# visanalexandru/felics

Hardware: AMD Instinct MI355X
Metric: encode MPix/s on 4K 8-bit grayscale batch (bit-exact); % HBM-read roofline (higher is better)
Workload: dtype u8

## Files before the change

### felics_amd/csrc/felics_kernels.hip

```cpp
#include <hip/hip_runtime.h>
#include <stdint.h>
#include <stdlib.h>
#include <string.h>
#include <type_traits>

#include "felics_device.h"
#include "felics_kernels.h"
#include "felics_codes.h"
#include "felics_pairs.h"

namespace felics {

thread_local LaunchTiming g_launch_timing;


__device__ __forceinline__ void ycocg(int r, int gr, int b, int &yv, int &co, int &cg) {
    co = r - b;
    const int t = b + co / 2;
    cg = gr - t;
    yv = t + cg / 2;
}

__device__ __forceinline__ void rgb8_group(const uint8_t *__restrict__ src, int16_t *__restrict__ o, uint32_t i, uint32_t npix, uint64_t stride) {
    if (i + 4 <= npix) {
        uint32_t w[3];
        __builtin_memcpy(w, src, 12);
        int yv[4], co[4], cg[4];
        ycocg((int)(w[0] & 0xFFu), (int)((w[0] >> 8) & 0xFFu), (int)((w[0] >> 16) & 0xFFu), yv[0], co[0], cg[0]);
        ycocg((int)(w[0] >> 24), (int)(w[1] & 0xFFu), (int)((w[1] >> 8) & 0xFFu), yv[1], co[1], cg[1]);
        ycocg((int)((w[1] >> 16) & 0xFFu), (int)(w[1] >> 24), (int)(w[2] & 0xFFu), yv[2], co[2], cg[2]);
        ycocg((int)((w[2] >> 8) & 0xFFu), (int)((w[2] >> 16) & 0xFFu), (int)(w[2] >> 24), yv[3], co[3], cg[3]);
        auto put4 = [&](int16_t *dst, const int (&v)[4]) {
            const uint32_t p[2] = {(uint32_t)(v[0] & 0xFFFF) | ((uint32_t)v[1] << 16),
                                   (uint32_t)(v[2] & 0xFFFF) | ((uint32_t)v[3] << 16)};
            __builtin_memcpy(dst, p, 8);
        };
        put4(o + i, yv);
        put4(o + stride + i, co);
        put4(o + 2ull * stride + i, cg);
    } else {
        for (uint32_t j = i; j < npix; j++) {
            int yv, co, cg;
            ycocg(src[(j - i) * 3], src[(j - i) * 3 + 1], src[(j - i) * 3 + 2], yv, co, cg);
            o[j] = (int16_t)yv;
            o[stride + j] = (int16_t)co;
            o[2ull * stride + j] = (int16_t)cg;
        }
    }
}
__global__ __launch_bounds__(256) void k_rgb8_to_planes(const uint8_t *__restrict__ rgb, int16_t *__restrict__ planes,
                                                        uint32_t npix, uint32_t nimg) {
    const uint32_t groups = (npix + 3) / 4;
    const uint64_t total = (uint64_t)groups * nimg;
    for (uint64_t g = (uint64_t)blockIdx.x * blockDim.x + threadIdx.x; g < total;
         g += (uint64_t)gridDim.x * blockDim.x) {
        const uint32_t img = (uint32_t)(g / groups);
        const uint32_t i = (uint32_t)(g - (uint64_t)img * groups) * 4;
        rgb8_group(rgb + ((uint64_t)img * npix + i) * 3, planes + (uint64_t)img * 3 * npix, i, npix, (uint64_t)npix);
    }
}
__global__ __launch_bounds__(256) void k_rgb8_to_planes_mixed(const PlaneGeom *__restrict__ table, uint64_t plane_stride) {
    const PlaneGeom *pg = table + 3ull * blockIdx.y;
    const uint32_t npix = pg->npix, groups = (npix + 3) / 4;
    const uint8_t *rgb = (const uint8_t *)pg->image;
    int16_t *o = (int16_t *)pg->samples;
    for (uint32_t g = blockIdx.x * blockDim.x + threadIdx.x; g < groups; g += gridDim.x * blockDim.x)
        rgb8_group(rgb + (uint64_t)g * 12u, o, g * 4, npix, plane_stride);
}

__global__ __launch_bounds__(256) void k_rgb8_view_to_planes(const PlaneGeom *__restrict__ table, const ViewRow *__restrict__ rows, uint64_t plane_stride) {
    const PlaneGeom *pg = table + 3ull * blockIdx.y;
    const ViewRow vr = rows[blockIdx.y];
    const uint32_t npix = pg->npix, W = pg->W, groups = (npix + 3) / 4;
    const uint8_t *data = (const uint8_t *)vr.data;
    const int64_t rs = vr.row_stride, ps = vr.pixel_stride, cs = vr.channel_stride;
    int16_t *o = (int16_t *)pg->samples;
    const bool unit = cs == 1 || cs == -1;
    const uint32_t mode = unit && ps == 3 ? 1u : unit && ps == 4 ? 2u : ps == 1 ? 3u : 0u;
    const uint8_t *low = data + (cs < 0 ? 2 * cs : 0);
    for (uint32_t g = blockIdx.x * blockDim.x + threadIdx.x; g < groups; g += gridDim.x * blockDim.x) {
        const uint32_t i = g * 4;
        uint32_t y = i / W, x = i - y * W;
        int r[4] = {0, 0, 0, 0}, gr[4] = {0, 0, 0, 0}, b[4] = {0, 0, 0, 0};
        const bool whole = i + 4 <= npix;
        const bool in_row = whole && x + 4 <= W && !(mode == 2u && x + 4 == W);
        if (in_row && mode == 1u) {
            uint32_t w[3];
            __builtin_memcpy(w, low + (int64_t)y * rs + (int64_t)x * 3, 12);
            const int q[12] = {(int)(w[0] & 0xFFu), (int)((w[0] >> 8) & 0xFFu), (int)((w[0] >> 16) & 0xFFu), (int)(w[0] >> 24),
                               (int)(w[1] & 0xFFu), (int)((w[1] >> 8) & 0xFFu), (int)((w[1] >> 16) & 0xFFu), (int)(w[1] >> 24),
                               (int)(w[2] & 0xFFu), (int)((w[2] >> 8) & 0xFFu), (int)((w[2] >> 16) & 0xFFu), (int)(w[2] >> 24)};
#pragma unroll
            for (uint32_t k = 0; k < 4; k++) {
                r[k] = cs > 0 ? q[3 * k] : q[3 * k + 2];
                gr[k] = q[3 * k + 1];
                b[k] = cs > 0 ? q[3 * k + 2] : q[3 * k];
            }
        } else if (in_row && mode == 2u) {
            uint32_t w[4];
            __builtin_memcpy(w, low + (int64_t)y * rs + (int64_t)x * 4, 16);
#pragma unroll
            for (uint32_t k = 0; k < 4; k++) {
                const int c0 = (int)(w[k] & 0xFFu), c2 = (int)((w[k] >> 16) & 0xFFu);
                r[k] = cs > 0 ? c0 : c2;
                gr[k] = (int)((w[k] >> 8) & 0xFFu);
                b[k] = cs > 0 ? c2 : c0;
            }
        } else if (in_row && mode == 3u) {
            const uint8_t *p = data + (int64_t)y * rs + (int64_t)x;
            load4(p, r);
            load4(p + cs, gr);
            load4(p + 2 * cs, b);
        } else {
            for (uint32_t k = 0; k < 4 && i + k < npix; k++) {
                const uint8_t *p = data + (int64_t)y * rs + (int64_t)x * ps;
                r[k] = p[0];
                gr[k] = p[cs];
                b[k] = p[2 * cs];
                if (++x == W) {
                    x = 0;
                    y++;
                }
            }
        }
        int yv[4], co[4], cg[4];
#pragma unroll
        for (uint32_t k = 0; k < 4; k++) ycocg(r[k], gr[k], b[k], yv[k], co[k], cg[k]);
        if (whole) {
            auto put4 = [&](int16_t *dst, const int (&v)[4]) {
                const uint32_t pk[2] = {(uint32_t)(v[0] & 0xFFFF) | ((uint32_t)v[1] << 16), (uint32_t)(v[2] & 0xFFFF) | ((uint32_t)v[3] << 16)};
                __builtin_memcpy(dst, pk, 8);
            };
            put4(o + i, yv);
            put4(o + plane_stride + i, co);
            put4(o + 2ull * plane_stride + i, cg);
        } else {
            for (uint32_t k = 0; i + k < npix; k++) {
                o[i + k] = (int16_t)yv[k];
                o[plane_stride + i + k] = (int16_t)co[k];
                o[2ull * plane_stride + i + k] = (int16_t)cg[k];
            }
        }
    }
}

template <uint32_t TABLE>
__device__ __forceinline__ uint32_t bitop3(uint32_t a, uint32_t b, uint32_t c) {
    return __builtin_amdgcn_bitop3_b32(a, b, c, TABLE);
}
constexpr uint32_t BT_SEL = 0xE4;
constexpr uint32_t BT_OR_ANDN = 0xF4;
constexpr uint32_t BT_ANDN = 0x30;
constexpr uint32_t BT_OR3 = 0xFE;
constexpr uint32_t BT_SEL_NOT = 0x72;
constexpr uint32_t BT_NOR = 0x03;
constexpr uint32_t BT_OR_AND = 0xF8;
__device__ __forceinline__ uint32_t min_u16(uint32_t a, uint32_t b) {
    uint32_t r;
    asm("v_min_u16 %0, %1, %2" : "=v"(r) : "v"(a), "v"(b));
    return r;
}
__device__ __forceinline__ uint32_t max_u16(uint32_t a, uint32_t b) {
    uint32_t r;
    asm("v_max_u16 %0, %1, %2" : "=v"(r) : "v"(a), "v"(b));
    return r;
}
template <uint32_t N>
__device__ __forceinline__ uint32_t shl_u16(uint32_t a) {
    uint32_t r;
    asm("v_lshlrev_b16 %0, %1, %2" : "=v"(r) : "n"(N), "v"(a));
    return r;
}
__device__ __forceinline__ uint32_t twice(uint32_t a) {
    uint32_t r;
    asm("v_add_u32 %0, %1, %1" : "=v"(r) : "v"(a));
    return r;
}
__device__ __forceinline__ uint32_t vgpr_const(uint32_t v) {
    uint32_t r;
    asm("v_mov_b32 %0, %1" : "=v"(r) : "s"(v));
    return r;
}

__device__ __forceinline__ uint32_t field_at(const uint32_t *w, uint32_t j, uint8_t) {
    const uint32_t x = w[j >> 2];
    switch (j & 3u) {
        case 0: return x & 0xFFu;
        case 1: {
            uint32_t r;
            asm("v_lshrrev_b16 %0, 8, %1" : "=v"(r) : "v"(x));
            return r;
        }
        case 2: return (x >> 16) & 0xFFu;
        default: return x >> 24;
    }
}
__device__ __forceinline__ uint32_t field_at(const uint32_t *w, uint32_t j, int16_t) {
    const uint32_t x = w[j >> 1] ^ 0x80008000u;
    return (j & 1u) ? x >> 16 : x & 0xFFFFu;
}
__device__ __forceinline__ uint32_t field_of(int v, uint8_t) { return (uint32_t)v & 0xFFu; }
__device__ __forceinline__ uint32_t field_of(int v, int16_t) { return ((uint32_t)v ^ 0x8000u) & 0xFFFFu; }

#ifndef FELICS_FORMS
#define FELICS_FORMS 255
#endif
#ifndef FELICS_FRONT_WAVES
#define FELICS_FRONT_WAVES 6
#endif
template <typename T>
struct PlaneView {
    const T *pl;
    uint32_t W, H, npix;
};
template <typename T>
__device__ __forceinline__ PlaneView<T> plane_view(const T *planes, uint32_t plane, uint32_t W, uint32_t npix) {
    return PlaneView<T>{planes + (uint64_t)plane * npix, W, 0u, npix};
}
template <typename T>
__device__ __forceinline__ PlaneView<T> plane_view(const PlaneGeom *table, uint32_t plane, uint32_t, uint32_t) {
    return plane_view<T>((const T *)nullptr, plane, table);
}
template <typename T>
__device__ __forceinline__ PlaneView<T> plane_view(const T *, uint32_t plane, const PlaneGeom *table) {
    const PlaneGeom *pg = table + (uint32_t)__builtin_amdgcn_readfirstlane((int)plane);
    return PlaneView<T>{(const T *)pg->samples, pg->W, pg->H, pg->npix};
}

template <typename T>
__device__ __forceinline__ PlaneView<T> plane_view(const PitchedGeom *rows, uint32_t plane, uint32_t, uint32_t) {
    const PitchedGeom *pg = rows + (uint32_t)__builtin_amdgcn_readfirstlane((int)plane);
    return PlaneView<T>{(const T *)pg->g.samples, pg->g.W, pg->g.H, pg->g.npix};
}
template <typename S>
__device__ __forceinline__ uint64_t plane_pitch(S, uint32_t) { return 0; }
__device__ __forceinline__ uint64_t plane_pitch(const PitchedGeom *rows, uint32_t plane) {
    return rows[(uint32_t)__builtin_amdgcn_readfirstlane((int)plane)].pitch;
}
#ifdef FELICS_FRONT_STAMPS
__device__ unsigned long long g_front_stamps[256][16];
#define FSTAMP(i)                                                              \
    do {                                                                       \
        const unsigned long long now_ = __builtin_amdgcn_s_memtime();          \
        f_acc[i] += now_ - f_last;                                             \
        f_last = now_;                                                         \
    } while (0)
#define FSTAMP_ARRIVED(d, t)                                                                                                              \
    do {                                                                                                                                  \
        FSTAMP(4 + (d));                                                                                                                  \
        asm volatile("" ::"v"(t.cur[0]), "v"(t.cur[1]), "v"(t.cur[2]), "v"(t.cur[3]), "v"(t.up[0]), "v"(t.up[1]), "v"(t.up[2]), "v"(t.up[3]), \
                     "v"(t.left0));                                                                                                       \
        FSTAMP(d);                                                                                                                        \
    } while (0)
#else
#define FSTAMP(i)
#define FSTAMP_ARRIVED(d, t)
#endif
template <typename T, typename ET, typename S, bool BALLOT>
__attribute__((amdgpu_waves_per_eu(sizeof(T) == 1 ? FELICS_FRONT_WAVES : 5))) __global__ __launch_bounds__(256) void k_front(
    S __restrict__ planes, ET *__restrict__ ev, uint16_t *__restrict__ pix, uint32_t *__restrict__ runtab,
    uint32_t *__restrict__ tile_slots, uint32_t W_, uint32_t npix_, uint32_t ntiles, uint32_t tile_begin, uint32_t tile_end,
    uint32_t nplanes, uint32_t cap, uint32_t *__restrict__ flags, uint32_t mode) {
    constexpr uint32_t NC = nctx_of<T>();
    constexpr uint32_t QUARTER = SORT_TILE / 4, TRIPS = QUARTER / 256;
    constexpr uint32_t PER = NC / 256;
    constexpr uint32_t KEY = 0xFFC00FFFu;
    static_assert(SORT_TILE % 1024 == 0 && SORT_TILE <= (1u << 12), "four whole trips per wave; 12 bits of pixel offset");
    static_assert(NC % 256 == 0 && NC <= 512, "a thread takes NC / 256 contexts; 9 bits of context");
    __shared__ uint32_t srt[SORT_TILE + 1 + 256];
    __shared__ uint32_t cnt[4][NC + 64];
    __shared__ uint32_t gdst[NC];
    __shared__ uint32_t wsum[4];
#ifdef FELICS_FRONT_STAMPS
    unsigned long long f_acc[15] = {}, f_last = __builtin_amdgcn_s_memtime();
#endif
    const uint32_t wave = (uint32_t)__builtin_amdgcn_readfirstlane((int)(threadIdx.x >> 6)), lane = lane_id();
    const uint32_t tid = threadIdx.x;
    const uint32_t wg_tiles = tile_end - tile_begin;
    const uint32_t item = blockIdx.x >> 3, xcd = blockIdx.x & 7u;
    const uint32_t plane = xcd + 8u * (item / wg_tiles);
    if (plane >= nplanes) return;
    const uint32_t tile = tile_begin + item % wg_tiles;
    uint32_t *my_cnt = cnt[wave];
    for (uint32_t c = lane; c < NC; c += 64) my_cnt[c] = 0;
    const PlaneView<T> view = plane_view<T>(planes, plane, W_, npix_);
    const uint32_t W = view.W, npix = view.npix;
    const T *pl = view.pl;
    constexpr bool PITCHED = std::is_same<S, const PitchedGeom *>::value;
    using Index = typename std::conditional<PITCHED, uint64_t, uint32_t>::type;
    const uint64_t pitch = plane_pitch(planes, plane);
    const uint32_t begin = tile * SORT_TILE;
    const uint32_t qbegin = min(begin + wave * QUARTER, npix);
    const uint32_t end = min(qbegin + QUARTER, npix);
    const bool safe_rank = (FELICS_FORMS & 1) ? BALLOT : (mode & FRONT_SAFE_RANK) != 0;
    constexpr uint32_t SLOTS = TRIPS * 4;
    uint32_t rec[SLOTS], rk[SLOTS];
    auto is_interior = [&](uint32_t r, uint32_t x, uint32_t y) { return y > 0 && x + 256 <= W && r + 256 <= end; };
    struct Trip {
        uint32_t cur[4], up[4], left0;
    };
    auto load_trip = [&](Index r, Index left_index, Trip &t) {
        if constexpr ((FELICS_FORMS & 2) != 0) {
            const T *row = pl + r, *above = row - W;
            if constexpr (PITCHED) above = row - pitch;
            uint32_t at = lane;
            asm volatile("" : "+v"(at));
#pragma unroll
            for (uint32_t j = 0; j < 4; j++) {
                t.cur[j] = field_of((int)(row + 64 * j)[at], T());
                t.up[j] = field_of((int)(above + 64 * j)[at], T());
            }
        } else {
#pragma unroll
            for (uint32_t j = 0; j < 4; j++) {
                t.cur[j] = field_of((int)pl[r + 64 * j + lane], T());
                if constexpr (PITCHED)
                    t.up[j] = field_of((int)pl[r + 64 * j + lane - pitch], T());
                else
                    t.up[j] = field_of((int)pl[r + 64 * j + lane - W], T());
            }
        }
        t.left0 = field_of((int)pl[left_index], T());
    };
    bool have[TRIPS];
    Index leftidx[TRIPS];
    Index tripat[TRIPS];
    {
        uint32_t ri = qbegin, yi = qbegin / W, xi = qbegin - yi * W;
#pragma unroll
        for (uint32_t d = 0; d < TRIPS; d++) {
            have[d] = ri < end && is_interior(ri, xi, yi);
            if constexpr (PITCHED) {
                tripat[d] = (uint64_t)yi * pitch + xi;
                leftidx[d] = !have[d] ? 0u : xi > 0 ? tripat[d] - 1 : (yi >= 2 ? tripat[d] - 2 * pitch : tripat[d] - pitch + 1);
            } else {
                leftidx[d] = have[d] ? span_left_index(ri, xi, yi, W) : 0u;
            }
            ri += 256;
            xi += 256;
            if (xi >= W) {
                const uint32_t q = xi / W;
                yi += q;
                xi -= q * W;
            }
        }
    }
    const uint32_t cnt_at = (uint32_t)(uintptr_t)(const __attribute__((address_space(3))) uint32_t *)my_cnt;
    const uint32_t dummy_at = (NC + lane) * 4u;
    constexpr uint32_t FLIGHT = (sizeof(T) == 1 && (FELICS_FORMS & 128) != 0) ? TRIPS : 2;
    static_assert(FLIGHT == 2 || FLIGHT == TRIPS, "two trips in turn, or all of the quarter's");
    Trip pre[FLIGHT];
    auto issue_trip = [&](uint32_t d) {
        if constexpr (PITCHED) {
            if (have[d]) load_trip(tripat[d], leftidx[d], pre[d % FLIGHT]);
        } else {
            if (have[d]) load_trip(qbegin + d * 256, leftidx[d], pre[d % FLIGHT]);
        }
    };
    if constexpr (FLIGHT == TRIPS) {
#pragma unroll
        for (uint32_t d = 0; d < TRIPS; d++) issue_trip(d);
    } else {
        issue_trip(0);
    }
    FSTAMP(11);
#pragma unroll
    for (uint32_t d = 0; d < TRIPS; d++) {
        const uint32_t row0 = qbegin + d * 256;
        if constexpr (FLIGHT != TRIPS) {
            if constexpr (PITCHED) {
                if (d + 1 < TRIPS && have[d + 1]) load_trip(tripat[d + 1], leftidx[d + 1], pre[(d + 1) & 1u]);
            } else {
                if (d + 1 < TRIPS && have[d + 1]) load_trip(row0 + 256, leftidx[d + 1], pre[(d + 1) & 1u]);
            }
        }
        if (have[d]) {
            const Trip &t = pre[d % FLIGHT];
            FSTAMP_ARRIVED(d, t);
#pragma unroll
            for (uint32_t j = 0; j < 4; j++) {
                uint32_t edge = t.left0;
                if (j > 0) edge = readlane(t.cur[j - 1], 63);
                const uint32_t a = (uint32_t)__builtin_amdgcn_update_dpp((int)edge, (int)t.cur[j], 0x138, 0xF, 0xF, false);
                const uint32_t p = t.cur[j], b = t.up[j];
                const uint32_t L = min_u16(a, b), H = max_u16(a, b);
                const uint32_t ctx = H - L;
                const int dd = (int)(p - L);
                const int below = dd >> 31;
                uint32_t val, in_range, above12, ctx4;
                if constexpr ((FELICS_FORMS & 4) != 0) {
                    const uint32_t t = H - p;
                    const uint32_t above = (uint32_t)((int)t >> 31);
                    val = bitop3<BT_SEL_NOT>((uint32_t)(dd ^ below), t, above);
                    in_range = bitop3<BT_NOR>(above, (uint32_t)below, 0u);
                    above12 = above & 0x1000u;
                    ctx4 = shl_u16<2>(ctx);
                } else {
                    const int o = (int)(p - H) - 1;
                    const int not_above = o >> 31;
                    val = bitop3<BT_SEL>((uint32_t)(dd ^ below), (uint32_t)o, (uint32_t)not_above);
                    in_range = bitop3<BT_ANDN>((uint32_t)not_above, (uint32_t)below, 0u);
                    above12 = bitop3<BT_ANDN>(0x1000u, (uint32_t)not_above, 0u);
                    ctx4 = ctx << 2;
                }
                const uint32_t off = row0 - begin + 64 * j + lane;
                if constexpr ((FELICS_FORMS & 4) != 0)
                    rec[d * 4 + j] = bitop3<BT_OR3>(bitop3<BT_OR3>(ctx << 22, val << 13, off), above12, in_range);
                else
                    rec[d * 4 + j] = ((ctx << 22) | (val << 13) | off | above12) | in_range;
                const uint32_t at = cnt_at + bitop3<BT_SEL>(dummy_at, ctx4, in_range);
                if (!safe_rank)
                    rk[d * 4 + j] = __hip_atomic_fetch_add((__attribute__((address_space(3))) uint32_t *)(uintptr_t)at, 1u, __ATOMIC_RELAXED, __HIP_MEMORY_SCOPE_WORKGROUP);
            }
        } else {
            Coord xy;
            xy.set(row0 + lane, W);
#pragma unroll
            for (uint32_t j = 0; j < 4; j++) {
                const uint32_t i = row0 + j * 64 + lane;
                uint32_t r = 0xFFFFFFFFu;
                if (i < end && i >= 2) {
                    PixelClass pc;
                    if constexpr (PITCHED)
                        pc = classify_pitched(pl, xy.x, xy.y, pitch);
                    else
                        pc = classify(pl, i, xy.x, xy.y, W);
                    if (pc.cls != CLS_IN) r = (pc.ctx << 22) | (pc.val << 13) | (pc.cls == CLS_ABOVE ? 0x1000u : 0u) | (i - begin);
                }
                xy.advance(64, W);
                rec[d * 4 + j] = r;
                const uint32_t at = cnt_at + ((int)r < 0 ? dummy_at : (r >> 22) << 2);
                if (!safe_rank)
                    rk[d * 4 + j] = __hip_atomic_fetch_add((__attribute__((address_space(3))) uint32_t *)(uintptr_t)at, 1u, __ATOMIC_RELAXED, __HIP_MEMORY_SCOPE_WORKGROUP);
            }
        }
        if (safe_rank) {
#pragma unroll
            for (uint32_t j = 0; j < 4; j++) {
                const bool e = (int)rec[d * 4 + j] >= 0;
                const uint32_t c = (rec[d * 4 + j] >> 22) & (NC - 1u);
                const uint64_t ev_mask = __ballot(e);
                uint32_t m_lo = (uint32_t)ev_mask, m_hi = (uint32_t)(ev_mask >> 32);
                constexpr uint32_t CTX_BITS = NC == 256 ? 8 : 9;
#pragma unroll
                for (uint32_t bt = 0; bt < CTX_BITS; bt++) {
                    const uint32_t tt = (uint32_t)((int32_t)(c << (31 - bt)) >> 31);
                    const uint64_t bb = __ballot(e && tt != 0);
                    m_lo &= ~((uint32_t)bb ^ tt);
                    m_hi &= ~((uint32_t)(bb >> 32) ^ tt);
                }
                const uint32_t rank = __builtin_amdgcn_mbcnt_hi(m_hi, __builtin_amdgcn_mbcnt_lo(m_lo, 0u));
                const uint32_t group = (uint32_t)__popc(m_lo) + (uint32_t)__popc(m_hi);
                uint32_t r = 0;
                if (e) r = my_cnt[c] + rank;
                __builtin_amdgcn_wave_barrier();
                if (e && rank == 0) my_cnt[c] = r + group;
                __builtin_amdgcn_wave_barrier();
                rk[d * 4 + j] = r;
            }
        }
    }
    FSTAMP(8);
    __syncthreads();
    FSTAMP(9);
    const uint64_t pt = (uint64_t)plane * ntiles + tile;
    uint32_t padpos[PER], nev_c[PER];
    {
        uint32_t n[4][PER], tot = 0;
#pragma unroll
        for (uint32_t u = 0; u < PER; u++) {
            nev_c[u] = 0;
#pragma unroll
            for (uint32_t w = 0; w < 4; w++) {
                n[w][u] = cnt[w][tid * PER + u];
                nev_c[u] += n[w][u];
            }
            tot += nev_c[u] | (((nev_c[u] + REC - 1u) & ~(REC - 1u)) << 16);
        }
        const uint32_t incl = wave_incl_scan(tot);
        if (lane == 63) wsum[wave] = incl;
        __syncthreads();
        uint32_t at = incl - tot;
        for (uint32_t w = 0; w < wave; w++) at += wsum[w];
#pragma unroll
        for (uint32_t u = 0; u < PER; u++) {
            const uint32_t c = tid * PER + u;
            uint32_t cs = at & 0xFFFFu;
            const uint32_t ps = at >> 16;
            padpos[u] = ps;
            gdst[c] = ps - cs;
#pragma unroll
            for (uint32_t w = 0; w < 4; w++) {
                cnt[w][c] = cs;
                cs += n[w][u];
            }
            at += nev_c[u] | (((nev_c[u] + REC - 1u) & ~(REC - 1u)) << 16);
        }
    }
    const uint32_t both = wsum[0] + wsum[1] + wsum[2] + wsum[3];
    const uint32_t total = both & 0xFFFFu, slots = both >> 16;
    if (tid == 0) srt[total] = 0xFFFFFFFFu;
    const bool fits = slots <= cap;
    if (fits) {
        uint32_t *rt = runtab + ((uint64_t)plane * NC + tid * PER) * ntiles + tile;
#pragma unroll
        for (uint32_t u = 0; u < PER; u++) rt[(uint64_t)u * ntiles] = (padpos[u] / REC) | (nev_c[u] << 16);
        uint16_t *px = pix + pt * cap;
#pragma unroll
        for (uint32_t u = 0; u < PER; u++)
            for (uint32_t i = nev_c[u]; i < ((nev_c[u] + REC - 1u) & ~(REC - 1u)); i++) px[padpos[u] + i] = 0xFFFFu;
        if (tid == 0) tile_slots[pt] = slots;
    } else {
        uint32_t *rt = runtab + ((uint64_t)plane * NC + tid * PER) * ntiles + tile;
#pragma unroll
        for (uint32_t u = 0; u < PER; u++) rt[(uint64_t)u * ntiles] = 0;
        if (tid == 0) {
            tile_slots[pt] = 0;
            atomicOr(flags, TL_FLAG_OVERFLOW);
        }
    }
    __syncthreads();
    FSTAMP(12);
#pragma unroll
    for (uint32_t q0 = 0; q0 < SLOTS; q0 += 8) {
        uint32_t at[8];
#pragma unroll
        for (uint32_t q = 0; q < 8; q++) at[q] = my_cnt[(rec[q0 + q] >> 22) & (NC - 1u)];
#pragma unroll
        for (uint32_t q = 0; q < 8; q++) {
            const uint32_t none = (uint32_t)((int)rec[q0 + q] >> 31);
            srt[bitop3<BT_SEL>(SORT_TILE + 1u + tid, at[q] + rk[q0 + q], none)] = rec[q0 + q];
        }
    }
    __syncthreads();
    FSTAMP(13);
    uint32_t bad = mode & FRONT_TEST_VIOLATION;
    if (fits) {
        ET *evo = ev + pt * cap;
        uint16_t *pxo = pix + pt * cap;
        for (uint32_t j = tid; j < total; j += 256) {
            const uint32_t r = srt[j], nxt = srt[j + 1];
            const uint32_t dst = gdst[r >> 22] + j;
            evo[dst] = (ET)((r >> 13) & 0x1FFu);
            pxo[dst] = (uint16_t)(r & 0x1FFFu);
            bad |= (nxt & KEY) <= (r & KEY) ? 1u : 0u;
        }
    }
    if (__ballot(bad != 0) != 0 && lane == 0) atomicOr(flags, TL_FLAG_ORDER);
#ifdef FELICS_FRONT_STAMPS
    FSTAMP(14);
    if (tid == 0) {
        unsigned long long *slot = g_front_stamps[(tile * 7u + plane) & 255u];
        for (int i = 0; i < 15; i++) atomicAdd(&slot[i], f_acc[i]);
        atomicAdd(&slot[15], 1ull);
    }
#endif
}

#ifdef FELICS_FRONT_STAMPS
extern "C" __attribute__((visibility("default"))) int felics_debug_front_stamps(unsigned long long *out, int reset) {
    if (hipMemcpyFromSymbol(out, HIP_SYMBOL(g_front_stamps), sizeof(g_front_stamps)) != hipSuccess) return -1;
    if (reset) {
        static unsigned long long z[256 * 16] = {};
        if (hipMemcpyToSymbol(HIP_SYMBOL(g_front_stamps), z, sizeof(z)) != hipSuccess) return -1;
    }
    return 0;
}
#endif



constexpr uint32_t STAGE_LEAD = 16;

template <typename T>
struct TileLDS {
    alignas(16) T cur[STAGE_LEAD + PACK_TILE];
    alignas(16) T up[PACK_TILE + 16];
    alignas(16) uint8_t kq[PACK_TILE];
    alignas(16) uint32_t dump[4];
};

template <typename U>
__device__ __forceinline__ void stage_span(U *lds, const U *__restrict__ g, int64_t first, uint32_t count,
                                           uint32_t limit) {
    constexpr uint32_t EPC = 16 / sizeof(U);
    const bool aligned = ((reinterpret_cast<uintptr_t>(g) + (uint64_t)first * sizeof(U)) & 15u) == 0;
    const uint32_t nchunks = (count + EPC - 1) / EPC;
    for (uint32_t c = threadIdx.x; c < nchunks; c += PACK_THREADS) {
        const int64_t g0 = first + (int64_t)c * EPC;
        if (aligned && g0 >= 0 && g0 + EPC <= (int64_t)limit) {
            reinterpret_cast<uint4 *>(lds)[c] = *reinterpret_cast<const uint4 *>(g + g0);
        } else {
#pragma unroll
            for (uint32_t e = 0; e < EPC; e++) {
                const int64_t gi = g0 + e;
                if (gi >= 0 && gi < (int64_t)limit && c * EPC + e < count) lds[c * EPC + e] = g[gi];
            }
        }
    }
}

template <typename T>
__device__ __forceinline__ void stage_pixels(TileLDS<T> &t, const T *__restrict__ pl, uint32_t tile_first, uint32_t W, uint32_t npix) {
    constexpr uint32_t EPC = 16 / sizeof(T);
    constexpr uint32_t NA = (STAGE_LEAD + PACK_TILE) / EPC, NB = (PACK_TILE + 16) / EPC;
    constexpr uint32_t KA = (NA + PACK_THREADS - 1) / PACK_THREADS, KB = (NB + PACK_THREADS - 1) / PACK_THREADS;
    static_assert((STAGE_LEAD + PACK_TILE) % EPC == 0 && (PACK_TILE + 16) % EPC == 0, "whole chunks");
    const int64_t fa = (int64_t)tile_first - STAGE_LEAD, fb = (int64_t)tile_first - W;
    const bool ala = ((reinterpret_cast<uintptr_t>(pl) + (uint64_t)fa * sizeof(T)) & 15u) == 0;
    const bool alb = ((reinterpret_cast<uintptr_t>(pl) + (uint64_t)fb * sizeof(T)) & 15u) == 0;
    const uint4 *safe = reinterpret_cast<const uint4 *>(pl - (reinterpret_cast<uintptr_t>(pl) & 15u) / sizeof(T));
    auto slowly = [&](T *lds, int64_t first, uint32_t c) {
        for (uint32_t e = 0; e < EPC; e++) {
            const int64_t gi = first + (int64_t)c * EPC + e;
            if (gi >= 0 && gi < (int64_t)npix) lds[c * EPC + e] = pl[gi];
        }
    };
    constexpr uint32_t FA = NA / PACK_THREADS, FB = NB / PACK_THREADS;
    static_assert(FA == FB && KA <= FA + 1 && KB <= FB + 1, "whole rounds, then at most one partial round");
    uint4 va[FA], vb[FB];
    bool wa[FA], wb[FB];
#pragma unroll
    for (uint32_t k = 0; k < FA; k++) {
        const uint32_t c = threadIdx.x + k * PACK_THREADS;
        const int64_t ga = fa + (int64_t)c * EPC, gb = fb + (int64_t)c * EPC;
        wa[k] = ala && ga >= 0 && ga + EPC <= (int64_t)npix;
        wb[k] = alb && gb >= 0 && gb + EPC <= (int64_t)npix;
        va[k] = *(wa[k] ? reinterpret_cast<const uint4 *>(pl + ga) : safe);
        vb[k] = *(wb[k] ? reinterpret_cast<const uint4 *>(pl + gb) : safe);
    }
    uint4 *dump = reinterpret_cast<uint4 *>(t.dump);
#pragma unroll
    for (uint32_t k = 0; k < FA; k++) {
        const uint32_t c = threadIdx.x + k * PACK_THREADS;
        *(wa[k] ? reinterpret_cast<uint4 *>(t.cur) + c : dump) = va[k];
        *(wb[k] ? reinterpret_cast<uint4 *>(t.up) + c : dump) = vb[k];
    }
#pragma unroll
    for (uint32_t k = 0; k < FA; k++) {
        const uint32_t c = threadIdx.x + k * PACK_THREADS;
        if (!wa[k]) slowly(t.cur, fa, c);
        if (!wb[k]) slowly(t.up, fb, c);
    }
    const uint32_t c1 = threadIdx.x + FA * PACK_THREADS;
    if (c1 < NA) {
        const int64_t g1 = fa + (int64_t)c1 * EPC;
        if (ala && g1 >= 0 && g1 + EPC <= (int64_t)npix) reinterpret_cast<uint4 *>(t.cur)[c1] = *reinterpret_cast<const uint4 *>(pl + g1);
        else slowly(t.cur, fa, c1);
    }
    if (c1 < NB) {
        const int64_t g1 = fb + (int64_t)c1 * EPC;
        if (alb && g1 >= 0 && g1 + EPC <= (int64_t)npix) reinterpret_cast<uint4 *>(t.up)[c1] = *reinterpret_cast<const uint4 *>(pl + g1);
        else slowly(t.up, fb, c1);
    }
}

template <typename T>
__device__ __forceinline__ void stage_tile(TileLDS<T> &t, const T *__restrict__ pl, const uint8_t *__restrict__ kpl,
                                           uint32_t tile_first, uint32_t W, uint32_t npix) {
    stage_span<T>(t.cur, pl, (int64_t)tile_first - STAGE_LEAD, STAGE_LEAD + PACK_TILE, npix);
    stage_span<T>(t.up, pl, (int64_t)tile_first - W, PACK_TILE + 16, npix);
    stage_span<uint8_t>(t.kq, kpl, (int64_t)tile_first, PACK_TILE, npix);
}
template <typename T>
__device__ __forceinline__ void stage_tile(TileLDS<T> &t, const T *__restrict__ pl, const uint8_t *__restrict__ kpl,
                                           uint32_t tile_first, uint32_t W, uint32_t npix, NoPitch) {
    stage_tile(t, pl, kpl, tile_first, W, npix);
}

template <typename U>
__device__ __forceinline__ void stage_span_pitched(U *lds, const U *__restrict__ g, int64_t first, uint32_t count, uint32_t limit,
                                                   uint32_t W, uint64_t pitch) {
    constexpr uint32_t EPC = 16 / sizeof(U);
    const uint32_t nchunks = (count + EPC - 1) / EPC;
    for (uint32_t c = threadIdx.x; c < nchunks; c += PACK_THREADS) {
        const int64_t g0 = first + (int64_t)c * EPC;
        if (g0 + (int64_t)EPC <= 0 || g0 >= (int64_t)limit) continue;
        const uint32_t i0 = (uint32_t)max(g0, (int64_t)0);
        Coord xy;
        xy.set(i0, W);
        const U *at = g + (uint64_t)xy.y * pitch + xy.x;
        if (g0 >= 0 && g0 + EPC <= (int64_t)limit && xy.x + EPC <= W && (reinterpret_cast<uintptr_t>(at) & 15u) == 0) {
            reinterpret_cast<uint4 *>(lds)[c] = *reinterpret_cast<const uint4 *>(at);
        } else {
            for (uint32_t e = (uint32_t)(i0 - g0); e < EPC; e++) {
                if (g0 + e >= (int64_t)limit || c * EPC + e >= count) break;
                lds[c * EPC + e] = g[(uint64_t)xy.y * pitch + xy.x];
                xy.advance(1, W);
            }
        }
    }
}
template <typename T>
__device__ __forceinline__ void stage_tile(TileLDS<T> &t, const T *__restrict__ pl, const uint8_t *__restrict__ kpl,
                                           uint32_t tile_first, uint32_t W, uint32_t npix, uint64_t pitch) {
    stage_span_pitched<T>(t.cur, pl, (int64_t)tile_first - STAGE_LEAD, STAGE_LEAD + PACK_TILE, npix, W, pitch);
    stage_span_pitched<T>(t.up, pl, (int64_t)tile_first - W, PACK_TILE + 16, npix, W, pitch);
    stage_span<uint8_t>(t.kq, kpl, (int64_t)tile_first, PACK_TILE, npix);
}
__device__ __forceinline__ uint64_t sample_index(uint32_t i, uint32_t, NoPitch) { return i; }
__device__ __forceinline__ uint64_t sample_index(uint32_t i, uint32_t W, uint64_t pitch) {
    const uint32_t y = i / W;
    return (uint64_t)y * pitch + (i - y * W);
}

template <typename T, typename FR, typename F, typename P = NoPitch>
__device__ __forceinline__ void walk_group(const TileLDS<T> &t, const uint8_t *kq, const T *__restrict__ pl, uint32_t first,
                                           uint32_t end, uint32_t W, FR &&raw, F &&f, P pitch = P{}) {
    if (first >= end) return;
    constexpr uint32_t NW = PACK_PER_THREAD * sizeof(T) / 4;
    const uint32_t off = threadIdx.x * PACK_PER_THREAD;
    uint32_t cw[NW], uw[NW], kw[4];
#pragma unroll
    for (uint32_t q = 0; q < NW / 4; q++) {
        const uint4 a = reinterpret_cast<const uint4 *>(t.cur + STAGE_LEAD + off)[q];
        const uint4 b = reinterpret_cast<const uint4 *>(t.up + off)[q];
        cw[4 * q] = a.x; cw[4 * q + 1] = a.y; cw[4 * q + 2] = a.z; cw[4 * q + 3] = a.w;
        uw[4 * q] = b.x; uw[4 * q + 1] = b.y; uw[4 * q + 2] = b.z; uw[4 * q + 3] = b.w;
    }
    {
        const uint4 c = *reinterpret_cast<const uint4 *>(kq + off);
        kw[0] = c.x; kw[1] = c.y; kw[2] = c.z; kw[3] = c.w;
    }
    int left = (int)t.cur[STAGE_LEAD + off - 1], left2 = (int)t.cur[STAGE_LEAD + off - 2];
    for (uint32_t i = first; i < min(end, 2u); i++) raw(i, (uint32_t)(int)pl[sample_index(i, W, pitch)]);
    Coord xy;
    xy.set(first, W);
    constexpr uint32_t D = sizeof(T);
    uint32_t up_tail = (uint32_t)(int)t.up[off + PACK_PER_THREAD];
#pragma nounroll
    for (uint32_t g = 0; g < PACK_PER_THREAD; g += 4) {
        const uint32_t un = NW > D ? uw[NW > D ? D : 0] : up_tail;
#pragma unroll
        for (uint32_t j = 0; j < 4; j++) {
            const uint32_t i = first + g + j;
            const int p = sample_at(cw, j, T());
            if (i < end && i >= 2) {
                const uint32_t k = (kw[0] >> (8u * j)) & 0xFFu;
                const int above = sample_at(uw, j, T());
                const bool row0 = xy.y == 0, col0 = xy.x == 0 && !row0;
                const int v1 = col0 ? above : left;
                int v2 = row0 ? left2 : above;
                if (col0) v2 = xy.y >= 2 ? (int)pl[sample_index(i - 2 * W, W, pitch)] : (j < 3 ? sample_at(uw, (j + 1) & 3u, T()) : sample_at(&un, 0, T()));
                const int H = max(v1, v2), L = min(v1, v2);
                const int d = p - L, ctx = H - L;
                const bool below = d < 0, over = d > ctx;
                PixelClass pc;
                pc.ctx = (uint32_t)ctx;
                pc.cls = (below ? (uint32_t)CLS_BELOW : 0u) | (over ? (uint32_t)CLS_ABOVE : 0u);
                uint32_t val = below ? (uint32_t)~d : (uint32_t)d;
                val = over ? (uint32_t)(d - ctx - 1) : val;
                pc.val = val;
                f(pc, k);
            }
            left2 = left;
            left = p;
            if (++xy.x == W) {
                xy.x = 0;
                xy.y++;
            }
        }
#pragma unroll
        for (uint32_t q = 0; q + D < NW; q++) {
            cw[q] = cw[q + D];
            uw[q] = uw[q + D];
        }
#pragma unroll
        for (uint32_t q = NW - D; q < NW; q++) uw[q] = up_tail;
        kw[0] = kw[1];
        kw[1] = kw[2];
        kw[2] = kw[3];
    }
}


template <typename T, bool MIXED, typename P = NoPitch>
__device__ __forceinline__ void lengths_tile(const T *__restrict__ pl, const uint8_t *__restrict__ kpl,
                                             group_bits_t<T> *__restrict__ group_bits, uint32_t *__restrict__ tile_bits, uint32_t W,
                                             uint32_t npix, uint32_t ntiles, uint32_t planes_per_image, uint32_t tile_begin, P pitch = P{}) {
    __shared__ TileLDS<T> tl;
    __shared__ uint32_t wsum[PACK_THREADS / 64];
    const uint32_t tile = tile_begin + blockIdx.x, plane = blockIdx.y;
    const uint32_t tile_first = tile * PACK_TILE;
    if constexpr (MIXED) {
        if (tile_first >= npix) {
            group_bits[((uint64_t)plane * ntiles + tile) * PACK_THREADS + threadIdx.x] = 0;
            if (threadIdx.x == 0) tile_bits[(uint64_t)plane * ntiles + tile] = 0;
            return;
        }
    }
    stage_tile(tl, pl, kpl, tile_first, W, npix, pitch);
    __syncthreads();
    const uint32_t first = tile_first + threadIdx.x * PACK_PER_THREAD;
    const uint32_t end = min(tile_first + PACK_TILE, npix);
    uint32_t bits = 0;
    walk_group(tl, tl.kq, pl, first, end, W, [&](uint32_t, uint32_t) { bits += 32u; },
               [&](const PixelClass &pc, uint32_t k) { bits += code_length(pc, k); }, pitch);
    if (npix == 1 && first == 0) bits += 32;
    if (tile == 0 && threadIdx.x == 0 && (plane % planes_per_image) == 0) bits += 8 * 14;
    group_bits[((uint64_t)plane * ntiles + tile) * PACK_THREADS + threadIdx.x] = (group_bits_t<T>)bits;
    const uint32_t inc = wave_incl_scan(bits);
    if (lane_id() == 63) wsum[threadIdx.x >> 6] = inc;
    __syncthreads();
    if (threadIdx.x == 0) {
        uint32_t tot = 0;
        for (uint32_t w = 0; w < PACK_THREADS / 64; w++) tot += wsum[w];
        tile_bits[(uint64_t)plane * ntiles + tile] = tot;
    }
}
template <typename T>
__global__ __launch_bounds__(PACK_THREADS) void k_lengths(const T *__restrict__ planes, const uint8_t *__restrict__ k_map,
                                                          group_bits_t<T> *__restrict__ group_bits,
                                                          uint32_t *__restrict__ tile_bits, uint32_t W, uint32_t npix,
                                                          uint32_t ntiles, uint32_t planes_per_image,
                                                          uint32_t tile_begin) {
    const uint32_t plane = blockIdx.y;
    lengths_tile<T, false>(planes + (uint64_t)plane * npix, k_map + (uint64_t)plane * npix, group_bits, tile_bits, W, npix, ntiles,
                           planes_per_image, tile_begin);
}
template <typename T>
__global__ __launch_bounds__(PACK_THREADS) void k_lengths_mixed(const PlaneGeom *__restrict__ table, const uint8_t *__restrict__ k_map,
                                                                group_bits_t<T> *__restrict__ group_bits,
                                                                uint32_t *__restrict__ tile_bits, uint32_t ntiles,
                                                                uint32_t planes_per_image, uint32_t tile_begin) {
    const uint32_t plane = blockIdx.y;
    const PlaneView<T> pv = plane_view<T>((const T *)nullptr, plane, table);
    lengths_tile<T, true>(pv.pl, k_map + (uint64_t)plane * ntiles * PACK_TILE, group_bits, tile_bits, pv.W, pv.npix, ntiles,
                          planes_per_image, tile_begin);
}
__global__ __launch_bounds__(PACK_THREADS) void k_lengths_pitched(const PitchedGeom16 *__restrict__ rows, const uint8_t *__restrict__ k_map,
                                                                  uint32_t *__restrict__ group_bits, uint32_t *__restrict__ tile_bits,
                                                                  uint32_t ntiles, uint32_t planes_per_image, uint32_t tile_begin) {
    const uint32_t plane = blockIdx.y;
    const PitchedGeom16 *pg = rows + (uint32_t)__builtin_amdgcn_readfirstlane((int)plane);
    lengths_tile<uint16_t, true, uint64_t>((const uint16_t *)pg->g.samples, k_map + (uint64_t)plane * ntiles * PACK_TILE, group_bits, tile_bits,
                                           pg->g.W, pg->g.npix, ntiles, planes_per_image, tile_begin, pg->pitch);
}


__global__ __launch_bounds__(1024) void k_bitscan_slice(const uint32_t *__restrict__ tile_bits,
// ... 1302 lines not shown
```

Measured before the change: 241,700.

## Scatter front records into padded slot order and emit vectorized packed outputs

```diff
diff --git a/felics_amd/csrc/felics_frontout.h b/felics_amd/csrc/felics_frontout.h
--- /dev/null
+++ b/felics_amd/csrc/felics_frontout.h
@@ -0,0 +1,67 @@
+#pragma once
+
+#include <stdint.h>
+
+#if defined(__HIPCC__)
+#define FELICS_FRONTOUT_FN __host__ __device__ __forceinline__
+#else
+#define FELICS_FRONTOUT_FN static inline
+#endif
+
+namespace felics {
+
+#if defined(__HIP_DEVICE_COMPILE__)
+FELICS_FRONTOUT_FN uint32_t frontout_perm(uint32_t hi, uint32_t lo, uint32_t sel) { return __builtin_amdgcn_perm(hi, lo, sel); }
+FELICS_FRONTOUT_FN uint32_t frontout_select(uint32_t a, uint32_t b, uint32_t c) { return __builtin_amdgcn_bitop3_b32(a, b, c, 0xE4); }
+#else
+FELICS_FRONTOUT_FN uint32_t frontout_select(uint32_t a, uint32_t b, uint32_t c) { return (a & c) | (b & ~c); }
+FELICS_FRONTOUT_FN uint32_t frontout_perm(uint32_t hi, uint32_t lo, uint32_t sel) {
+    const uint64_t src = ((uint64_t)hi << 32) | lo;
+    uint32_t r = 0;
+    for (uint32_t i = 0; i < 4; i++) {
+        const uint32_t s = (sel >> (8 * i)) & 0xFFu;
+        uint32_t b;
+        if (s <= 7) b = (uint32_t)(src >> (8 * s)) & 0xFFu;
+        else if (s <= 11) b = ((src >> (16 * (s - 8) + 15)) & 1u) ? 0xFFu : 0u;
+        else b = s == 12 ? 0u : 0xFFu;
+        r |= b << (8 * i);
+    }
+    return r;
+}
+#endif
+
+constexpr uint32_t FRONTOUT_KEY = 0xFFC00FFFu;
+constexpr uint32_t FRONTOUT_PAD = 0xFFFFFFFFu;
+constexpr uint32_t FRONTOUT_REC = 16;
+
+FELICS_FRONTOUT_FN uint32_t frontout_pix_pair(uint32_t r0, uint32_t r1) {
+    const uint32_t low = frontout_perm(r1, r0, 0x05040100u);
+    const uint32_t pad = frontout_perm(r1, r0, 0x0b0b0909u);
+    return frontout_select(low, pad, 0x1FFF1FFFu);
+}
+FELICS_FRONTOUT_FN uint32_t frontout_ev_u8(uint32_t r0, uint32_t r1, uint32_t r2, uint32_t r3) {
+    const uint32_t lo = frontout_perm(r1 >> 13, r0 >> 13, 0x0c0c0400u);
+    const uint32_t hi = frontout_perm(r3 >> 13, r2 >> 13, 0x04000c0cu);
+    return lo | hi;
+}
+FELICS_FRONTOUT_FN uint32_t frontout_ev_u16(uint32_t r0, uint32_t r1) {
+    return frontout_perm(r1 >> 13, r0 >> 13, 0x05040100u) & 0x01FF01FFu;
+}
+
+FELICS_FRONTOUT_FN uint32_t frontout_key(uint32_t e) { return e | ~FRONTOUT_KEY; }
+FELICS_FRONTOUT_FN bool frontout_pair_bad(uint32_t r, uint32_t nxt) { return frontout_key(nxt) < frontout_key(r) + 1u; }
+
+FELICS_FRONTOUT_FN uint32_t frontout_layout_term(uint32_t events) {
+    return events | (((events + FRONTOUT_REC - 1u) & ~(FRONTOUT_REC - 1u)) << 16);
+}
+FELICS_FRONTOUT_FN void frontout_slot_bases(uint32_t sums_in_front, const uint32_t (&n)[4], uint32_t (&cursor)[4]) {
+    uint32_t at = sums_in_front >> 16;
+    for (uint32_t w = 0; w < 4; w++) {
+        cursor[w] = at;
+        at += n[w];
+    }
+}
+
+FELICS_FRONTOUT_FN bool frontout_one_window(uint32_t slots, uint32_t window) { return slots <= window; }
+
+}
diff --git a/felics_amd/csrc/felics_kernels.hip b/felics_amd/csrc/felics_kernels.hip
--- a/felics_amd/csrc/felics_kernels.hip
+++ b/felics_amd/csrc/felics_kernels.hip
@@ -8,6 +8,7 @@
 #include "felics_kernels.h"
 #include "felics_codes.h"
 #include "felics_pairs.h"
+#include "felics_frontout.h"
 
 namespace felics {
 
@@ -203,7 +204,7 @@
 __device__ __forceinline__ uint32_t field_of(int v, int16_t) { return ((uint32_t)v ^ 0x8000u) & 0xFFFFu; }
 
 #ifndef FELICS_FORMS
-#define FELICS_FORMS 255
+#define FELICS_FORMS 511
 #endif
 #ifndef FELICS_FRONT_WAVES
 #define FELICS_FRONT_WAVES 6
@@ -265,9 +266,11 @@
     constexpr uint32_t QUARTER = SORT_TILE / 4, TRIPS = QUARTER / 256;
     constexpr uint32_t PER = NC / 256;
     constexpr uint32_t KEY = 0xFFC00FFFu;
+    static_assert(KEY == felics::FRONTOUT_KEY && REC == felics::FRONTOUT_REC, "felics_frontout.h speaks of the same record");
     static_assert(SORT_TILE % 1024 == 0 && SORT_TILE <= (1u << 12), "four whole trips per wave; 12 bits of pixel offset");
     static_assert(NC % 256 == 0 && NC <= 512, "a thread takes NC / 256 contexts; 9 bits of context");
-    __shared__ uint32_t srt[SORT_TILE + 1 + 256];
+    constexpr bool SLOT_ORDER = (FELICS_FORMS & 256) != 0;
+    __shared__ alignas(16) uint32_t srt[SORT_TILE + 1 + 256];
     __shared__ uint32_t cnt[4][NC + 64];
     __shared__ uint32_t gdst[NC];
     __shared__ uint32_t wsum[4];
@@ -460,11 +463,17 @@
             }
         }
     }
+    if constexpr (SLOT_ORDER) {
+#pragma unroll
+        for (uint32_t k = 0; k < SORT_TILE / 1024; k++) reinterpret_cast<uint4 *>(srt)[k * 256 + tid] = make_uint4(~0u, ~0u, ~0u, ~0u);
+        if (tid == 0) srt[SORT_TILE] = 0xFFFFFFFFu;
+    }
     FSTAMP(8);
     __syncthreads();
     FSTAMP(9);
     const uint64_t pt = (uint64_t)plane * ntiles + tile;
     uint32_t padpos[PER], nev_c[PER];
+    bool in_slots = false;
     {
         uint32_t n[4][PER], tot = 0;
 #pragma unroll
@@ -475,40 +484,52 @@
                 n[w][u] = cnt[w][tid * PER + u];
                 nev_c[u] += n[w][u];
             }
-            tot += nev_c[u] | (((nev_c[u] + REC - 1u) & ~(REC - 1u)) << 16);
+            tot += felics::frontout_layout_term(nev_c[u]);
         }
         const uint32_t incl = wave_incl_scan(tot);
         if (lane == 63) wsum[wave] = incl;
         __syncthreads();
         uint32_t at = incl - tot;
         for (uint32_t w = 0; w < wave; w++) at += wsum[w];
+        if constexpr (SLOT_ORDER) in_slots = felics::frontout_one_window((wsum[0] + wsum[1] + wsum[2] + wsum[3]) >> 16, SORT_TILE);
 #pragma unroll
         for (uint32_t u = 0; u < PER; u++) {
             const uint32_t c = tid * PER + u;
             uint32_t cs = at & 0xFFFFu;
             const uint32_t ps = at >> 16;
             padpos[u] = ps;
-            gdst[c] = ps - cs;
-#pragma unroll
-            for (uint32_t w = 0; w < 4; w++) {
-                cnt[w][c] = cs;
-                cs += n[w][u];
-            }
-            at += nev_c[u] | (((nev_c[u] + REC - 1u) & ~(REC - 1u)) << 16);
+            if (SLOT_ORDER && in_slots) {
+                const uint32_t nw[4] = {n[0][u], n[1][u], n[2][u], n[3][u]};
+                uint32_t cursor[4];
+                felics::frontout_slot_bases(at, nw, cursor);
+#pragma unroll
+                for (uint32_t w = 0; w < 4; w++) cnt[w][c] = cursor[w];
+            } else {
+                gdst[c] = ps - cs;
+#pragma unroll
+                for (uint32_t w = 0; w < 4; w++) {
+                    cnt[w][c] = cs;
+                    cs += n[w][u];
+                }
+            }
+            at += felics::frontout_layout_term(nev_c[u]);
         }
     }
     const uint32_t both = wsum[0] + wsum[1] + wsum[2] + wsum[3];
     const uint32_t total = both & 0xFFFFu, slots = both >> 16;
-    if (tid == 0) srt[total] = 0xFFFFFFFFu;
+    if (!in_slots)
+        if (tid == 0) srt[total] = 0xFFFFFFFFu;
     const bool fits = slots <= cap;
     if (fits) {
         uint32_t *rt = runtab + ((uint64_t)plane * NC + tid * PER) * ntiles + tile;
 #pragma unroll
         for (uint32_t u = 0; u < PER; u++) rt[(uint64_t)u * ntiles] = (padpos[u] / REC) | (nev_c[u] << 16);
-        uint16_t *px = pix + pt * cap;
-#pragma unroll
-        for (uint32_t u = 0; u < PER; u++)
-            for (uint32_t i = nev_c[u]; i < ((nev_c[u] + REC - 1u) & ~(REC - 1u)); i++) px[padpos[u] + i] = 0xFFFFu;
+        if (!in_slots) {
+            uint16_t *px = pix + pt * cap;
+#pragma unroll
+            for (uint32_t u = 0; u < PER; u++)
+                for (uint32_t i = nev_c[u]; i < ((nev_c[u] + REC - 1u) & ~(REC - 1u)); i++) px[padpos[u] + i] = 0xFFFFu;
+        }
         if (tid == 0) tile_slots[pt] = slots;
     } else {
         uint32_t *rt = runtab + ((uint64_t)plane * NC + tid * PER) * ntiles + tile;
@@ -535,7 +556,30 @@
     __syncthreads();
     FSTAMP(13);
     uint32_t bad = mode & FRONT_TEST_VIOLATION;
-    if (fits) {
+    if (SLOT_ORDER && in_slots) {
+        if (fits) {
+            char *evo = reinterpret_cast<char *>(ev + pt * cap);
+            char *pxo = reinterpret_cast<char *>(pix + pt * cap);
+            bool unordered = false;
+            for (uint32_t g = tid; 4u * g < slots; g += 256u) {
+                uint32_t g_ = g;
+                asm volatile("" : "+v"(g_));
+                const uint32_t j = 4u * g_;
+                uint4 e = *reinterpret_cast<const uint4 *>(&srt[j]);
+                const uint32_t nxt = srt[j + 4u];
+                asm volatile("" : "+v"(e.x), "+v"(e.y), "+v"(e.z), "+v"(e.w));
+                if constexpr (sizeof(ET) == 1)
+                    *reinterpret_cast<uint32_t *>(evo + j) = felics::frontout_ev_u8(e.x, e.y, e.z, e.w);
+                else
+                    *reinterpret_cast<uint2 *>(evo + 2u * j) = make_uint2(felics::frontout_ev_u16(e.x, e.y), felics::frontout_ev_u16(e.z, e.w));
+                *reinterpret_cast<uint2 *>(pxo + 2u * j) = make_uint2(felics::frontout_pix_pair(e.x, e.y), felics::frontout_pix_pair(e.z, e.w));
+                const bool b0 = felics::frontout_pair_bad(e.x, e.y), b1 = felics::frontout_pair_bad(e.y, e.z);
+                const bool b2 = felics::frontout_pair_bad(e.z, e.w), b3 = felics::frontout_pair_bad(e.w, nxt);
+                unordered |= b0 | b1 | b2 | b3;
+            }
+            bad |= unordered ? 1u : 0u;
+        }
+    } else if (fits) {
         ET *evo = ev + pt * cap;
         uint16_t *pxo = pix + pt * cap;
         for (uint32_t j = tid; j < total; j += 256) {
diff --git a/felics_amd/csrc/frontout_check.cpp b/felics_amd/csrc/frontout_check.cpp
--- /dev/null
+++ b/felics_amd/csrc/frontout_check.cpp
@@ -0,0 +1,239 @@
+#include <stdint.h>
+#include <stdio.h>
+#include <string.h>
+
+#include <vector>
+
+#include "felics_frontout.h"
+
+using namespace felics;
+
+namespace {
+
+constexpr uint32_t WINDOW = 4096, PASS = 1024;
+
+uint64_t failures = 0;
+void fail(const char *what, uint64_t a, uint64_t b, uint64_t got, uint64_t want) {
+    if (failures++ < 20) fprintf(stderr, "frontout_check: %s (%#llx, %#llx): %#llx, expected %#llx\n", what, (unsigned long long)a, (unsigned long long)b,
+                                 (unsigned long long)got, (unsigned long long)want);
+}
+
+uint32_t entry(uint32_t ctx, uint32_t val, uint32_t above, uint32_t off) { return ctx << 22 | val << 13 | above << 12 | off; }
+uint32_t ref_pix(uint32_t r) { return r == FRONTOUT_PAD ? 0xFFFFu : ((r >> 12) & 1u) << 12 | (r & 0xFFFu); }
+uint32_t ref_val(uint32_t r) { return (r >> 13) & 0x1FFu; }
+bool ref_bad(uint32_t r, uint32_t nxt) {
+    if (r == FRONTOUT_PAD || nxt == FRONTOUT_PAD) return false;
+    const uint32_t c0 = r >> 22, c1 = nxt >> 22, o0 = r & 0xFFFu, o1 = nxt & 0xFFFu;
+    return c1 < c0 || (c1 == c0 && o1 <= o0);
+}
+
+const uint32_t OFFS[] = {0, 1, 2, 63, 64, 255, 256, 0x7FF, 0x800, 0xFFE, 0xFFF};
+const uint32_t CTXS[] = {0, 1, 2, 127, 128, 254, 255, 256, 257, 510, 511};
+
+uint64_t check_words() {
+    uint64_t n = 0;
+    std::vector<uint32_t> partners = {FRONTOUT_PAD, 0u, entry(511, 511, 1, 0xFFF), entry(255, 255, 0, 0x800), entry(256, 1, 1, 1)};
+    for (uint32_t ctx = 0; ctx < 512; ctx++)
+        for (uint32_t val = 0; val < 512; val++)
+            for (uint32_t off : OFFS)
+                for (uint32_t above = 0; above < 2; above++) {
+                    const uint32_t r = entry(ctx, val, above, off);
+                    for (uint32_t q : partners) {
+                        const uint32_t a = frontout_pix_pair(r, q), b = frontout_pix_pair(q, r);
+                        if (a != (ref_pix(r) | ref_pix(q) << 16)) fail("pix word, low half", r, q, a, ref_pix(r) | ref_pix(q) << 16);
+                        if (b != (ref_pix(q) | ref_pix(r) << 16)) fail("pix word, high half", q, r, b, ref_pix(q) | ref_pix(r) << 16);
+                        const uint32_t e = frontout_ev_u16(r, q), f = frontout_ev_u16(q, r);
+                        if ((e & 0xFFFFu) != ref_val(r)) fail("ev word (u16), low half", r, q, e, ref_val(r));
+                        if ((f >> 16) != ref_val(r)) fail("ev word (u16), high half", q, r, f, ref_val(r));
+                        if (q != FRONTOUT_PAD && (e >> 16) != ref_val(q)) fail("ev word (u16), partner", r, q, e, ref_val(q));
+                        if (val < 256 && ctx < 256) {
+                            for (uint32_t pos = 0; pos < 4; pos++) {
+                                uint32_t four[4] = {q, q, q, q};
+                                four[pos] = r;
+                                const uint32_t w = frontout_ev_u8(four[0], four[1], four[2], four[3]);
+                                if (((w >> (8 * pos)) & 0xFFu) != val) fail("ev word (u8)", r, pos, w, val);
+                                if (q != FRONTOUT_PAD && ((w >> (8 * (pos ^ 1u))) & 0xFFu) != (ref_val(q) & 0xFFu)) fail("ev word (u8), partner", q, pos, w, ref_val(q));
+                            }
+                        }
+                        n++;
+                    }
+                }
+    if (frontout_pix_pair(FRONTOUT_PAD, FRONTOUT_PAD) != 0xFFFFFFFFu) fail("pix word of two padding slots", 0, 0, frontout_pix_pair(FRONTOUT_PAD, FRONTOUT_PAD), 0xFFFFFFFFu);
+    return n;
+}
+
+uint64_t check_pairs() {
+    uint64_t n = 0;
+    std::vector<uint32_t> es = {FRONTOUT_PAD};
+    for (uint32_t c : CTXS)
+        for (uint32_t o : OFFS)
+            for (uint32_t va = 0; va < 4; va++) es.push_back(entry(c, va & 1u ? 511u : 0u, va >> 1, o));
+    for (uint32_t r : es)
+        for (uint32_t nx : es) {
+            if (frontout_pair_bad(r, nx) != ref_bad(r, nx)) fail("order predicate", r, nx, frontout_pair_bad(r, nx), ref_bad(r, nx));
+            n++;
+        }
+    return n;
+}
+
+struct Tile {
+    uint32_t nctx;
+    std::vector<uint32_t> n[4];
+};
+struct Event {
+    uint32_t rec, wave, rank;
+};
+
+bool run_tile(const Tile &t, uint32_t swap_at, std::vector<uint16_t> &pix, std::vector<uint16_t> &ev, uint32_t &slots_out) {
+    std::vector<Event> events;
+    std::vector<uint32_t> cursor[4];
+    uint32_t sums = 0, off = 0;
+    for (uint32_t w = 0; w < 4; w++) cursor[w].resize(t.nctx);
+    std::vector<uint32_t> off_of[4];
+    for (uint32_t w = 0; w < 4; w++) {
+        off_of[w].resize(t.nctx);
+        for (uint32_t c = 0; c < t.nctx; c++) {
+            off_of[w][c] = off;
+            off += t.n[w][c];
+        }
+    }
+    if (off > 4096) fail("the generator made more than 4096 events", off, 0, off, 4096);
+    for (uint32_t c = 0; c < t.nctx; c++) {
+        const uint32_t nw[4] = {t.n[0][c], t.n[1][c], t.n[2][c], t.n[3][c]};
+        uint32_t cur[4];
+        frontout_slot_bases(sums, nw, cur);
+        for (uint32_t w = 0; w < 4; w++) {
+            cursor[w][c] = cur[w];
+            for (uint32_t k = 0; k < nw[w]; k++) events.push_back(Event{entry(c, (c + k) & 0x1FFu, k & 1u, (off_of[w][c] + k) & 0xFFFu), w, k});
+        }
+        sums += frontout_layout_term(nw[0] + nw[1] + nw[2] + nw[3]);
+    }
+    const uint32_t slots = sums >> 16;
+    slots_out = slots;
+    if (swap_at != ~0u) {
+        Event *a = nullptr, *b = nullptr;
+        for (Event &e : events) {
+            const uint32_t s = cursor[e.wave][e.rec >> 22] + e.rank;
+            if (s == swap_at) a = &e;
+            if (s == swap_at + 1) b = &e;
+        }
+        if (!a || !b || a->wave != b->wave || (a->rec >> 22) != (b->rec >> 22)) return false;
+        const uint32_t k = a->rank;
+        a->rank = b->rank;
+        b->rank = k;
+    }
+    if (!frontout_one_window(slots, WINDOW)) return false;
+    pix.assign(slots, 0x1234);
+    ev.assign(slots, 0x1234);
+    std::vector<uint32_t> srt(WINDOW + 1 + 1, FRONTOUT_PAD);
+    for (const Event &e : events) srt[cursor[e.wave][e.rec >> 22] + e.rank] = e.rec;
+    bool bad = false;
+    for (uint32_t p0 = 0; p0 < slots; p0 += PASS)
+        for (uint32_t j = p0; j < p0 + PASS && j < slots; j += 4) {
+            const uint32_t *e = &srt[j];
+            const uint32_t p01 = frontout_pix_pair(e[0], e[1]), p23 = frontout_pix_pair(e[2], e[3]);
+            const uint32_t v01 = frontout_ev_u16(e[0], e[1]), v23 = frontout_ev_u16(e[2], e[3]);
+            const uint32_t ps[4] = {p01 & 0xFFFFu, p01 >> 16, p23 & 0xFFFFu, p23 >> 16}, vs[4] = {v01 & 0xFFFFu, v01 >> 16, v23 & 0xFFFFu, v23 >> 16};
+            for (uint32_t i = 0; i < 4; i++) {
+                pix[j + i] = (uint16_t)ps[i];
+                ev[j + i] = (uint16_t)vs[i];
+                bad |= frontout_pair_bad(e[i], e[i + 1]);
+            }
+        }
+    if (srt[WINDOW] != FRONTOUT_PAD) fail("the word behind the last slot", slots, 0, srt[WINDOW], FRONTOUT_PAD);
+    return bad;
+}
+
+void ref_tile(const Tile &t, std::vector<uint16_t> &pix, std::vector<uint16_t> &ev) {
+    pix.clear();
+    ev.clear();
+    uint32_t off = 0;
+    std::vector<uint32_t> off_of[4];
+    for (uint32_t w = 0; w < 4; w++) {
+        off_of[w].resize(t.nctx);
+        for (uint32_t c = 0; c < t.nctx; c++) {
+            off_of[w][c] = off;
+            off += t.n[w][c];
+        }
+    }
+    for (uint32_t c = 0; c < t.nctx; c++) {
+        for (uint32_t w = 0; w < 4; w++)
+            for (uint32_t k = 0; k < t.n[w][c]; k++) {
+                pix.push_back((uint16_t)(((off_of[w][c] + k) & 0xFFFu) | (k & 1u) << 12));
+                ev.push_back((uint16_t)((c + k) & 0x1FFu));
+            }
+        while (pix.size() % FRONTOUT_REC) {
+            pix.push_back(0xFFFF);
+            ev.push_back(0xFFFF);
+        }
+    }
+}
+
+uint64_t exchanges = 0, large = 0;
+uint64_t check_tiles() {
+    uint64_t n = 0;
+    for (uint32_t mark : {1024u, 2048u, 4096u})
+        for (uint32_t gap = 0; gap <= 3; gap++)
+            for (uint32_t len = 0; len <= 33; len++)
+                for (uint32_t split = 0; split < 3; split++)
+                    for (uint32_t len2 : {0u, 1u, 16u, 33u}) {
+                        const uint32_t lead = mark / FRONTOUT_REC - gap;
+                        Tile t;
+                        t.nctx = 512;
+                        for (uint32_t w = 0; w < 4; w++) t.n[w].assign(t.nctx, 0);
+                        uint32_t c = 0, left = lead;
+                        while (left) {
+                            const uint32_t recs = c < 20 ? 2u : 1u;
+                            const uint32_t evs = recs == 2 ? 17u : 1u + (c * 5u) % 16u;
+                            for (uint32_t k = 0; k < evs; k++) t.n[(k * 7 + c) & 3u][c]++;
+                            left -= recs;
+                            c++;
+                        }
+                        const uint32_t cu = c + 3;
+                        for (uint32_t k = 0; k < len; k++) t.n[split == 0 ? 0u : split == 1 ? (k & 3u) : (k < len / 2 ? 1u : 3u)][cu]++;
+                        for (uint32_t k = 0; k < len2; k++) t.n[(k + 1) & 3u][cu + 1]++;
+                        if (cu + 1 >= t.nctx) {
+                            fail("the generator ran out of contexts", lead, cu, cu, t.nctx);
+                            continue;
+                        }
+                        std::vector<uint16_t> pix, ev, rpix, rev;
+                        uint32_t slots = 0;
+                        const bool bad = run_tile(t, ~0u, pix, ev, slots);
+                        ref_tile(t, rpix, rev);
+                        if (!frontout_one_window(slots, WINDOW)) {
+                            if (rpix.size() <= WINDOW || slots != rpix.size()) fail("a tile taken for large", lead, len, slots, rpix.size());
+                            large++;
+                            continue;
+                        }
+                        if (bad) fail("order check fired on a sorted tile", lead, len, 1, 0);
+                        if (pix.size() != rpix.size()) fail("slots in use", lead, len, pix.size(), rpix.size());
+                        else
+                            for (size_t s = 0; s < pix.size(); s++) {
+                                if (pix[s] != rpix[s]) fail("pix of slot", s, len, pix[s], rpix[s]);
+                                if (rpix[s] != 0xFFFF && ev[s] != rev[s]) fail("ev of slot", s, len, ev[s], rev[s]);
+                            }
+                        for (uint32_t s = mark - 72; s < mark + 72 && s + 1 < slots; s++) {
+                            std::vector<uint16_t> p2, e2;
+                            uint32_t s2 = 0;
+                            const bool caught = run_tile(t, s, p2, e2, s2);
+                            if (p2.empty()) continue;
+                            if (!caught) fail("exchanged neighbours not caught at slot", s, len, 0, 1);
+                            exchanges++;
+                        }
+                        n++;
+                    }
+    return n;
+}
+
+}
+
+int main() {
+    const uint64_t words = check_words(), pairs = check_pairs(), tiles = check_tiles();
+    if (failures) {
+        fprintf(stderr, "frontout_check: %llu mismatches\n", (unsigned long long)failures);
+        return 1;
+    }
+    printf("frontout_check: %llu entry classes beside their partners, %llu ordered pairs, %llu tiles at the pass boundaries and the window's end (and %llu larger), %llu exchanges caught: ok\n",
+           (unsigned long long)words, (unsigned long long)pairs, (unsigned long long)tiles, (unsigned long long)large, (unsigned long long)exchanges);
+    return 0;
+}
```

After: 244,600, median of 6. 1.2% higher.
